# jai1215snu/ShiftedScaleQuantization

Measured on AMD Instinct MI355X. Metric: Gelem/s shifted-scale q/dq + recon iters/s, ResNet-18 W2A4; top-1 vs ref, higher is better.
Workload: dtype f32; 1 GPU; resnet18 W2A4 bias_cal+bias_ch_quant, 1024 calib samples: A4 per-tensor q/dq of act [1024,64,56,56] + W2 per-channel q/dq of all 21 conv/fc weights (8-bit stem/head); parallelism=dp1

## Files before the change

### shiftedscalequantization_amd/csrc/conv_wgrad.hip

```cpp
#include <stdlib.h>

#include <algorithm>
#include <type_traits>

#include "ssq_common.h"

namespace ssq {

typedef float f32x16 __attribute__((ext_vector_type(16)));

constexpr int kUnr = 2;

struct WgradGeo {
  int Nb, C, H, W, Co, OH, OW, R, S, st, pad, G, Cig, Cog;
  int Ncol;
  int WM;
  int Pq;
  int lda;
  int chunks_per_n;
  int nchunks;
  int cps;
  int nsplit;
  int in_rows;
  int ci_span;
// ... 1071 lines not shown
  WgradGeo g;
  size_t lds;
  return wgrad_plan(Nb, C, H, W, Co, R, S, stride, pad, groups, g, &lds) ? 0 : 1;
}

extern "C" size_t ssq_conv_wgrad_workspace_size(int64_t Nb, int64_t C, int64_t H, int64_t W,
                                                int64_t Co, int64_t R, int64_t S, int64_t stride,
                                                int64_t pad, int64_t groups) {
  if (is_depthwise(C, Co, groups) && R * S <= 25 && Nb >= 1 && dw_lds_ok(H, W, pad)) {
    int spl;
    const int ns = dw_splits(Nb, C, &spl);
    const int64_t OH = (H + 2 * pad - R) / stride + 1;
    int64_t nbands = 1;
    if (dw_stage(H, W, pad, spl) == 0 && OH >= 1) {
      const int bh = dw_band_rows(H, W, R, stride, pad, OH);
      nbands = (OH + bh - 1) / bh;
    }
    return (size_t)ns * (size_t)nbands * (size_t)C * (size_t)(R * S) * sizeof(float);
  }
  {
    BandGeo gb;
    int wmx, vpx;
    if (use_band(Nb, C, H, W, Co, R, S, stride, pad, groups, gb, &wmx, &vpx))
      return (size_t)gb.nsplit * 9 * (size_t)Co * (size_t)C * sizeof(float);
  }
  if (use_i2c(R, S, Co, groups)) {
    I2cGeo gi;
    int wm;
    if (wgrad_i2c_plan(Nb, C, H, W, Co, R, S, stride, pad, groups, gi)) return 0;
    wgrad_i2c_tiles(gi, &wm);
    return (size_t)gi.nsplit * (size_t)Co * (size_t)gi.Ncol * sizeof(float);
  }
  if (R == 1 && S == 1 && pad == 0) {
    W1Geo g1;
    if (wgrad_1x1_plan(Nb, C, H, W, Co, stride, groups, g1)) return 0;
    return (size_t)g1.nsplit * (size_t)Co * (size_t)g1.Cig * sizeof(float);
  }
  WgradGeo g;
  size_t lds;
  if (wgrad_plan(Nb, C, H, W, Co, R, S, stride, pad, groups, g, &lds)) return 0;
  return (size_t)g.nsplit * (size_t)Co * (size_t)g.Ncol * sizeof(float);
}

extern "C" int ssq_conv_wgrad(const float* x, const float* dy, int64_t Nb, int64_t C, int64_t H,
                              int64_t W, int64_t Co, int64_t R, int64_t S, int64_t stride,
                              int64_t pad, int64_t groups, float* dw, void* ws, size_t ws_bytes,
                              ssq_stream_t stream) {
  SSQ_REQUIRE(x && dy && dw, SSQ_E_ARG, "ssq_conv_wgrad: null pointer");
  hipStream_t s = (hipStream_t)stream;
  if (is_depthwise(C, Co, groups) && R * S <= 25 && dw_lds_ok(H, W, pad)) {
    SSQ_REQUIRE(Nb >= 1 && H >= 1 && W >= 1 && stride >= 1 && pad >= 0, SSQ_E_ARG,
                "ssq_conv_wgrad: bad geometry");
    const int64_t OH = (H + 2 * pad - R) / stride + 1, OW = (W + 2 * pad - S) / stride + 1;
    SSQ_REQUIRE(OH >= 1 && OW >= 1 && Nb * C * H * W < (1ll << 31) && Nb * C * OH * OW < (1ll << 31),
                SSQ_E_ARG, "ssq_conv_wgrad: sizes");
    int spl;
    const int ns = dw_splits(Nb, C, &spl);
    const size_t need = (size_t)ns * (size_t)C * (size_t)(R * S) * sizeof(float);
    SSQ_REQUIRE(ws && ws_bytes >= need, SSQ_E_WS, "ssq_conv_wgrad: workspace too small");
    const dim3 grid((unsigned)C, (unsigned)ns);
    const int64_t plane = (H + 2 * pad) * (W + 2 * pad);
    const int nb = dw_stage(H, W, pad, spl);
    if (nb > 0) {
      const size_t lds = (size_t)nb * plane * sizeof(float);
      const FastDiv dWp = make_fastdiv((uint32_t)(W + 2 * pad)), dP = make_fastdiv((uint32_t)plane),
                    dOHW = make_fastdiv((uint32_t)(OH * OW)), dOW = make_fastdiv((uint32_t)OW);
      if (R * S <= 9)
        hipLaunchKernelGGL(wgrad_dw_small<9>, grid, dim3(256), lds, s, x, dy, (int)C, (int)H,
                           (int)W, (int)OH, (int)OW, (int)R, (int)S, (int)stride, (int)pad, spl,
                           nb, dWp, dP, dOHW, dOW, (float*)ws);
      else
        hipLaunchKernelGGL(wgrad_dw_small<25>, grid, dim3(256), lds, s, x, dy, (int)C, (int)H,
                           (int)W, (int)OH, (int)OW, (int)R, (int)S, (int)stride, (int)pad, spl,
                           nb, dWp, dP, dOHW, dOW, (float*)ws);
      const int64_t n = C * R * S;
      hipLaunchKernelGGL(wgrad_stage2, dim3((unsigned)std::min<int64_t>((n + 63) / 64, 4096)),
                         dim3(256), 0, s, (const float*)ws, ns, n, dw);
      return check_launch("ssq_conv_wgrad");
    }
    const int bh = dw_band_rows(H, W, R, stride, pad, OH);
    const int nbands = (int)((OH + bh - 1) / bh);
    SSQ_REQUIRE(ws_bytes >= need * (size_t)nbands, SSQ_E_WS, "ssq_conv_wgrad: workspace too small");
    const dim3 gridb((unsigned)C, (unsigned)(ns * nbands));
    const size_t lds = (size_t)(((int64_t)bh - 1) * stride + R) * (W + 2 * pad) * sizeof(float);
    static bool dw_attr = false;
    if (!dw_attr) {
      hipFuncSetAttribute((const void*)wgrad_dw_stage1<9>,
                          hipFuncAttributeMaxDynamicSharedMemorySize, 128 * 1024);
      hipFuncSetAttribute((const void*)wgrad_dw_stage1<25>,
                          hipFuncAttributeMaxDynamicSharedMemorySize, 128 * 1024);
      dw_attr = true;
    }
    if (R * S <= 9)
      hipLaunchKernelGGL(wgrad_dw_stage1<9>, gridb, dim3(256), lds, s, x, dy, (int)C, (int)H, (int)W,
                         (int)OH, (int)OW, (int)R, (int)S, (int)stride, (int)pad, spl, bh, nbands,
                         make_fastdiv((uint32_t)(W + 2 * pad)), (float*)ws);
    else
      hipLaunchKernelGGL(wgrad_dw_stage1<25>, gridb, dim3(256), lds, s, x, dy, (int)C, (int)H, (int)W,
                         (int)OH, (int)OW, (int)R, (int)S, (int)stride, (int)pad, spl, bh, nbands,
                         make_fastdiv((uint32_t)(W + 2 * pad)), (float*)ws);
    const int64_t n = C * R * S;
    hipLaunchKernelGGL(wgrad_stage2, dim3((unsigned)std::min<int64_t>((n + 63) / 64, 4096)),
                       dim3(256), 0, s, (const float*)ws, ns * nbands, n, dw);
    return check_launch("ssq_conv_wgrad");
  }
  {
    BandGeo gb;
    int wmx, vpx;
    if (use_band(Nb, C, H, W, Co, R, S, stride, pad, groups, gb, &wmx, &vpx)) {
      const size_t needb = (size_t)gb.nsplit * 9 * (size_t)Co * (size_t)C * sizeof(float);
      SSQ_REQUIRE(ws && ws_bytes >= needb, SSQ_E_WS, "ssq_conv_wgrad: workspace too small");
      typedef void (*BandK)(const float*, const float*, BandGeo, float*);
#define SSQ_BK(NWV)                                                                          \
  {{{wgrad_band_stage1<2, 1, 4, NWV>, wgrad_band_stage1<2, 1, 2, NWV>,                        \
     wgrad_band_stage1<2, 1, 1, NWV>},                                                        \
    {wgrad_band_stage1<2, 2, 4, NWV>, wgrad_band_stage1<2, 2, 2, NWV>,                        \
     wgrad_band_stage1<2, 2, 1, NWV>}},                                                       \
   {{wgrad_band_stage1<4, 1, 4, NWV>, wgrad_band_stage1<4, 1, 2, NWV>,                        \
     wgrad_band_stage1<4, 1, 1, NWV>},                                                        \
    {wgrad_band_stage1<4, 2, 4, NWV>, wgrad_band_stage1<4, 2, 2, NWV>,                        \
     wgrad_band_stage1<4, 2, 1, NWV>}}}
      static const BandK kernels[2][2][2][3] = {SSQ_BK(4), SSQ_BK(8)};
#undef SSQ_BK
      static bool band_attr = false;
      if (!band_attr) {
        for (auto& a0 : kernels)
          for (auto& a : a0)
            for (auto& b : a)
              for (BandK k : b)
                hipFuncSetAttribute((const void*)k, hipFuncAttributeMaxDynamicSharedMemorySize,
                                    160 * 1024);
        band_attr = true;
      }
      const int w8 = band_waves() == 8;
      const BandK kb = kernels[w8][wmx == 4][stride == 2][vpx == 4 ? 0 : (vpx == 2 ? 1 : 2)];
      const dim3 gridb((unsigned)(gb.nsplit * gb.m_tiles * gb.n_tiles));
      const size_t ldsb = 2 * (size_t)gb.bufsz * sizeof(float);
      hipLaunchKernelGGL(kb, gridb, dim3(w8 ? 512 : 256), ldsb, s, x, dy, gb, (float*)ws);
      const int64_t inner = Co * C, nb = 9 * inner;
      hipLaunchKernelGGL(wgrad_stage2, dim3((unsigned)std::min<int64_t>((nb + 63) / 64, 4096)),
                         dim3(256), 0, s, (const float*)ws, gb.nsplit, nb, dw, inner, 9);
      return check_launch("ssq_conv_wgrad");
    }
  }
  if (use_i2c(R, S, Co, groups)) {
    I2cGeo gi;
    int wm;
    const int rci = wgrad_i2c_plan(Nb, C, H, W, Co, R, S, stride, pad, groups, gi);
    if (rci) return rci;
    wgrad_i2c_tiles(gi, &wm);
    const size_t needi = (size_t)gi.nsplit * (size_t)Co * (size_t)gi.Ncol * sizeof(float);
    SSQ_REQUIRE(ws && ws_bytes >= needi, SSQ_E_WS, "ssq_conv_wgrad: workspace too small");
    const dim3 gridi(gi.n_tiles, gi.m_tiles * gi.G, gi.nsplit);
    (void)wm;
    hipLaunchKernelGGL(wgrad_i2c_stage1<2>, gridi, dim3(256), 0, s, x, dy, gi, (float*)ws);
    const int64_t ni = (int64_t)Co * gi.Ncol;
    hipLaunchKernelGGL(wgrad_stage2, dim3((unsigned)std::min<int64_t>((ni + 63) / 64, 4096)),
                       dim3(256), 0, s, (const float*)ws, gi.nsplit, ni, dw);
    return check_launch("ssq_conv_wgrad");
  }
  if (R == 1 && S == 1 && pad == 0) {
    W1Geo g1;
    const int rc1 = wgrad_1x1_plan(Nb, C, H, W, Co, stride, groups, g1);
    if (rc1) return rc1;
    const size_t need1 = (size_t)g1.nsplit * (size_t)Co * (size_t)g1.Cig * sizeof(float);
    SSQ_REQUIRE(ws && ws_bytes >= need1, SSQ_E_WS, "ssq_conv_wgrad: workspace too small");
    const dim3 grid1(g1.n_tiles, g1.m_tiles * g1.G, g1.nsplit);
    hipLaunchKernelGGL(wgrad_1x1_stage1<2>, grid1, dim3(256), 0, s, x, dy, g1, (float*)ws);
    const int64_t n1 = (int64_t)Co * g1.Cig;
    hipLaunchKernelGGL(wgrad_stage2, dim3((unsigned)std::min<int64_t>((n1 + 63) / 64, 4096)),
                       dim3(256), 0, s, (const float*)ws, g1.nsplit, n1, dw);
    return check_launch("ssq_conv_wgrad");
  }
  WgradGeo g;
  size_t lds;
  int rc = wgrad_plan(Nb, C, H, W, Co, R, S, stride, pad, groups, g, &lds);
  if (rc) return rc;
  const size_t need = (size_t)g.nsplit * (size_t)Co * (size_t)g.Ncol * sizeof(float);
  SSQ_REQUIRE(ws && ws_bytes >= need, SSQ_E_WS, "ssq_conv_wgrad: workspace too small");
  static bool lds_attr = false;
  if (!lds_attr) {
    hipFuncSetAttribute((const void*)wgrad_stage1<1>, hipFuncAttributeMaxDynamicSharedMemorySize,
                        160 * 1024);
    hipFuncSetAttribute((const void*)wgrad_stage1<2>, hipFuncAttributeMaxDynamicSharedMemorySize,
                        160 * 1024);
    hipFuncSetAttribute((const void*)wgrad_stage1<4>, hipFuncAttributeMaxDynamicSharedMemorySize,
                        160 * 1024);
    lds_attr = true;
  }
  const dim3 grid(g.n_tiles, g.m_tiles * g.G, g.nsplit);
  if (g.WM == 1)
    hipLaunchKernelGGL(wgrad_stage1<1>, grid, dim3(256), lds, s, x, dy, g, (float*)ws);
  else if (g.WM == 2)
    hipLaunchKernelGGL(wgrad_stage1<2>, grid, dim3(256), lds, s, x, dy, g, (float*)ws);
  else
    hipLaunchKernelGGL(wgrad_stage1<4>, grid, dim3(256), lds, s, x, dy, g, (float*)ws);
  const int64_t n = (int64_t)Co * g.Ncol;
  hipLaunchKernelGGL(wgrad_stage2, dim3((unsigned)std::min<int64_t>((n + 63) / 64, 4096)),
                     dim3(256), 0, s, (const float*)ws, g.nsplit, n, dw);
  return check_launch("ssq_conv_wgrad");
}

__global__ __launch_bounds__(kBlock) void wgrad_gemm_operands(
    const float* __restrict__ x, const float* __restrict__ dy, uint32_t C, uint32_t H,
    uint32_t W, uint32_t Co, uint32_t R, uint32_t S, uint32_t st, int pad, uint32_t OW,
    uint32_t NP, FastDiv dRS, FastDiv dS, FastDiv dP, FastDiv dOW, uint32_t CRS,
    uint32_t P, uint32_t nb1, uint32_t tiles_k, uint32_t vec4, float* __restrict__ col,
    float* __restrict__ dy2) {
  if (blockIdx.x < nb1) {
    __shared__ float tile[64][65];
    const uint32_t tk = blockIdx.x % tiles_k, tp = blockIdx.x / tiles_k;
    const uint32_t row0 = tp * 64, k0 = tk * 64, RS = R * S;
    const uint32_t pp = threadIdx.x & 63, kb = threadIdx.x >> 6, row = row0 + pp;
    const bool rok = row < NP;
    const uint32_t n = rok ? fdiv(row, dP) : 0u, p = row - n * P;
    const uint32_t oh = fdiv(p, dOW), ow = p - oh * OW;
    const int ih0 = (int)(oh * st) - pad, iw0 = (int)(ow * st) - pad;
    const float* xn = x + (size_t)n * C * H * W;
    float v[16];
#pragma unroll
    for (int j = 0; j < 16; ++j) {
      const uint32_t k = k0 + kb + 4 * j;
      const uint32_t ci = fdiv(k, dRS), rs = k - ci * RS;
      const uint32_t r = fdiv(rs, dS), sc = rs - r * S;
      const int ih = ih0 + (int)r, iw = iw0 + (int)sc;
      v[j] = 0.0f;
      if (rok && k < CRS && ih >= 0 && ih < (int)H && iw >= 0 && iw < (int)W)
        v[j] = xn[((size_t)ci * H + ih) * W + iw];
    }
#pragma unroll
    for (int j = 0; j < 16; ++j) tile[kb + 4 * j][pp] = v[j];
    __syncthreads();
    if (vec4) {
      for (uint32_t i = threadIdx.x; i < 64 * 16; i += kBlock) {
        const uint32_t pp = i >> 4, kq = (i & 15) << 2;
        const uint32_t row = row0 + pp, k = k0 + kq;
        if (row < NP && k < CRS)
          *reinterpret_cast<float4*>(col + (size_t)row * CRS + k) =
              make_float4(tile[kq][pp], tile[kq + 1][pp], tile[kq + 2][pp], tile[kq + 3][pp]);
      }
    } else {
      for (uint32_t i = threadIdx.x; i < 64 * 64; i += kBlock) {
        const uint32_t pp = i >> 6, kk = i & 63;
        const uint32_t row = row0 + pp, k = k0 + kk;
        if (row < NP && k < CRS) col[(size_t)row * CRS + k] = tile[kk][pp];
      }
    }
    return;
  }
  const uint32_t nb2 = gridDim.x - nb1;
  const uint32_t n2 = Co * NP;
  for (uint32_t e = (blockIdx.x - nb1) * kBlock + threadIdx.x; e < n2; e += nb2 * kBlock) {
    const uint32_t co = e / NP, q = e - co * NP;
    const uint32_t n = fdiv(q, dP), p = q - n * P;
    dy2[e] = dy[((size_t)n * Co + co) * P + p];
  }
}

template <int ACT>
__device__ __forceinline__ float epi_in(float v, uint32_t c, const float* __restrict__ bias,
                                        const float* __restrict__ gamma,
                                        const float* __restrict__ phi, bool quant,
                                        const QParams& qp) {
  float t = bias ? __fadd_rn(v, bias[c]) : v;
  if (gamma) t = __fadd_rn(__fmul_rn(t, gamma[c]), phi[c]);
  t = act_fwd<ACT>(t);
  if (quant) {
    float q;
    t = fq1(t, qp, &q);
  }
  return t;
}

template <int ACT>
__global__ __launch_bounds__(kBlock) void gemm_col_epi(
    const float* __restrict__ y, const float* __restrict__ bias, const float* __restrict__ gamma,
    const float* __restrict__ phi, const float* __restrict__ qdelta,
    const float* __restrict__ qzp, float qlo, float qhi, uint32_t C, uint32_t H, uint32_t W,
    uint32_t R, uint32_t S, uint32_t st, int pad, uint32_t OW, uint32_t NP, FastDiv dCRS,
    FastDiv dRS, FastDiv dS, FastDiv dP, FastDiv dOW, uint32_t CRS, uint32_t P,
    float* __restrict__ col) {
  const bool quant = qdelta != nullptr;
  QParams qp{1.0f, 0.0f, qlo, qhi};
  if (quant) {
    qp.d = qdelta[0];
    qp.z = qzp[0];
  }
  const uint32_t n1 = NP * CRS;
  for (uint32_t e = blockIdx.x * kBlock + threadIdx.x; e < n1; e += gridDim.x * kBlock) {
    const uint32_t row = fdiv(e, dCRS), k = e - row * CRS;
    const uint32_t n = fdiv(row, dP), p = row - n * P;
    const uint32_t oh = fdiv(p, dOW), ow = p - oh * OW;
    const uint32_t ci = fdiv(k, dRS), rs = k - ci * R * S;
    const uint32_t r = fdiv(rs, dS), s = rs - r * S;
    const int ih = (int)(oh * st + r) - pad, iw = (int)(ow * st + s) - pad;
    float v = 0.0f;
    if (ih >= 0 && ih < (int)H && iw >= 0 && iw < (int)W)
      v = epi_in<ACT>(y[(((size_t)n * C + ci) * H + ih) * W + iw], ci, bias, gamma, phi, quant,
                      qp);
    col[e] = v;
  }
}

extern "C" int ssq_gemm_col_epilogue(const float* y, const float* bias, const float* gamma,
                                     const float* phi, int relu, const float* delta,
                                     const float* zp, int qmin, int qmax, int64_t Nb, int64_t C,
                                     int64_t H, int64_t W, int64_t R, int64_t S, int64_t stride,
                                     int64_t pad, float* col, ssq_stream_t stream) {
  SSQ_REQUIRE(y && col, SSQ_E_ARG, "ssq_gemm_col_epilogue: null pointer");
  SSQ_REQUIRE(!gamma == !phi, SSQ_E_ARG, "ssq_gemm_col_epilogue: gamma and phi go together");
  SSQ_REQUIRE(!delta || (zp && qmin < qmax), SSQ_E_ARG, "ssq_gemm_col_epilogue: act quantizer");
  SSQ_REQUIRE(relu >= 0 && relu <= 2, SSQ_E_ARG, "ssq_gemm_col_epilogue: activation code %d", relu);
  SSQ_REQUIRE(Nb >= 1 && C >= 1 && H >= 1 && W >= 1 && R >= 1 && S >= 1 && stride >= 1 &&
                  pad >= 0, SSQ_E_ARG, "ssq_gemm_col_epilogue: bad geometry");
  const int64_t OH = (H + 2 * pad - R) / stride + 1, OW = (W + 2 * pad - S) / stride + 1;
  SSQ_REQUIRE(OH >= 1 && OW >= 1, SSQ_E_ARG, "ssq_gemm_col_epilogue: empty output plane");
  const int64_t P = OH * OW, NP = Nb * P, CRS = C * R * S;
  SSQ_REQUIRE(NP * CRS < (1ll << 31) && Nb * C * H * W < (1ll << 31), SSQ_E_ARG,
              "ssq_gemm_col_epilogue: operands exceed 2^31 elements");
  const uint32_t nb = (uint32_t)std::min<int64_t>((NP * CRS + kBlock - 1) / kBlock, 8192);
#define SSQ_GCE(A)                                                                          \
  hipLaunchKernelGGL(gemm_col_epi<A>, dim3(nb), dim3(kBlock), 0, (hipStream_t)stream, y, bias, \
                     gamma, phi, delta, zp, (float)qmin, (float)qmax, (uint32_t)C, (uint32_t)H, \
                     (uint32_t)W, (uint32_t)R, (uint32_t)S, (uint32_t)stride, (int)pad,         \
                     (uint32_t)OW, (uint32_t)NP, make_fastdiv((uint32_t)CRS),                   \
                     make_fastdiv((uint32_t)(R * S)), make_fastdiv((uint32_t)S),                \
                     make_fastdiv((uint32_t)P), make_fastdiv((uint32_t)OW), (uint32_t)CRS,      \
                     (uint32_t)P, col)
  if (relu == 2) SSQ_GCE(2); else if (relu == 1) SSQ_GCE(1); else SSQ_GCE(0);
#undef SSQ_GCE
  return check_launch("ssq_gemm_col_epilogue");
}

extern "C" int ssq_wgrad_gemm_operands(const float* x, const float* dy, int64_t Nb, int64_t C,
                                       int64_t H, int64_t W, int64_t Co, int64_t R, int64_t S,
                                       int64_t stride, int64_t pad, float* col, float* dy2,
                                       ssq_stream_t stream) {
  SSQ_REQUIRE((x && col) || (dy && dy2), SSQ_E_ARG, "ssq_wgrad_gemm_operands: null pointer");
  if (!(x && col)) col = nullptr;
  if (!(dy && dy2)) dy2 = nullptr;
  SSQ_REQUIRE(Nb >= 1 && C >= 1 && H >= 1 && W >= 1 && Co >= 1 && R >= 1 && S >= 1 &&
                  stride >= 1 && pad >= 0, SSQ_E_ARG, "ssq_wgrad_gemm_operands: bad geometry");
  const int64_t OH = (H + 2 * pad - R) / stride + 1, OW = (W + 2 * pad - S) / stride + 1;
  SSQ_REQUIRE(OH >= 1 && OW >= 1, SSQ_E_ARG, "ssq_wgrad_gemm_operands: empty output plane");
  const int64_t P = OH * OW, NP = Nb * P, CRS = C * R * S;
  SSQ_REQUIRE(NP * CRS < (1ll << 31) && Co * NP < (1ll << 31) && Nb * C * H * W < (1ll << 31),
              SSQ_E_ARG, "ssq_wgrad_gemm_operands: operands exceed 2^31 elements");
  const bool vec4 = col && CRS % 4 == 0 && ((uintptr_t)col & 15) == 0;
  const int64_t tiles_k = (CRS + 63) / 64, tiles = ((NP + 63) / 64) * tiles_k;
  SSQ_REQUIRE(tiles < (1ll << 31), SSQ_E_ARG, "ssq_wgrad_gemm_operands: too many tiles");
  const uint32_t nb1 = col ? (uint32_t)tiles : 0u;
  const uint32_t nb2 = dy2 ? (uint32_t)std::min<int64_t>((Co * NP + kBlock - 1) / kBlock, 2048) : 0u;
  hipLaunchKernelGGL(wgrad_gemm_operands, dim3(nb1 + nb2), dim3(kBlock), 0, (hipStream_t)stream,
                     x, dy, (uint32_t)C, (uint32_t)H, (uint32_t)W, (uint32_t)Co, (uint32_t)R,
                     (uint32_t)S, (uint32_t)stride, (int)pad, (uint32_t)OW, (uint32_t)NP,
                     make_fastdiv((uint32_t)(R * S)), make_fastdiv((uint32_t)S),
                     make_fastdiv((uint32_t)P), make_fastdiv((uint32_t)OW), (uint32_t)CRS,
                     (uint32_t)P, nb1, (uint32_t)tiles_k, (uint32_t)vec4, col, dy2);
  return check_launch("ssq_wgrad_gemm_operands");
}
```

Measured before the change: 753.9 Gelem/s.

## Stage input planes in LDS for im2col with fused epilogue and dy repack

Adds a col_staged kernel that loads padded input channel-block bands into shared memory, applies the activation/quant epilogue once per input element, and then emits im2col rows from LDS using vectorized float4 stores. It also folds the dy-to-dy2 repack into the same launch with a vectorized copy path. The goal is to stop re-reading and re-quantizing each input element R*S times from global memory during im2col for wgrad and the GEMM epilogue. In exchange it adds occupancy-sensitive LDS use, env-driven planning heuristics and a fallback for 1x1 or strided cases.

```diff
diff --git a/shiftedscalequantization_amd/csrc/conv_wgrad.hip b/shiftedscalequantization_amd/csrc/conv_wgrad.hip
--- a/shiftedscalequantization_amd/csrc/conv_wgrad.hip
+++ b/shiftedscalequantization_amd/csrc/conv_wgrad.hip
@@ -1397,6 +1397,282 @@
   }
 }
 
+struct ColPlan {
+  uint32_t Nb, C, H, W, R, S, st, OH, OW, P, CRS, RS;
+  int pad;
+  uint32_t CB, NS, BH;
+  uint32_t ncb, nbands;
+  uint32_t Wp, PS;
+  uint32_t vec_in, vec_out;
+  uint32_t nb1;
+  FastDiv dRS, dS, dOW, dBH, dW;
+};
+
+struct Dy2Plan {
+  uint32_t Co, P, NP, chunks, vec;
+  FastDiv dP, dChunks;
+};
+
+struct EpiArgs {
+  const float *bias, *gamma, *phi, *qdelta, *qzp;
+  float qlo, qhi;
+};
+
+constexpr uint32_t kColCB = 32;
+constexpr size_t kColLdsCap = 48 * 1024;
+constexpr size_t kColPlaneCap = 160 * 1024;
+
+template <int EPI>
+__global__ __launch_bounds__(kBlock) void col_staged(const float* __restrict__ x, ColPlan g,
+                                                     EpiArgs ea, float* __restrict__ col,
+                                                     const float* __restrict__ dy, Dy2Plan d,
+                                                     float* __restrict__ dy2) {
+  extern __shared__ __align__(16) float col_lds[];
+  const uint32_t t = threadIdx.x;
+  if (blockIdx.x >= g.nb1) {
+    const uint32_t b2 = blockIdx.x - g.nb1, co = fdiv(b2, d.dChunks);
+    const uint32_t q0 = (b2 - co * d.chunks) * (4 * kBlock);
+    const float* src = dy + (size_t)co * d.P;
+    float* dst = dy2 + (size_t)co * d.NP;
+    if (d.vec) {
+      const uint32_t q = q0 + 4 * t;
+      if (q < d.NP) {
+        const uint32_t n = fdiv(q, d.dP), p = q - n * d.P;
+        *reinterpret_cast<float4*>(dst + q) =
+            *reinterpret_cast<const float4*>(src + (size_t)n * d.Co * d.P + p);
+      }
+    } else {
+#pragma unroll
+      for (int j = 0; j < 4; ++j) {
+        const uint32_t q = q0 + t + kBlock * j;
+        if (q < d.NP) {
+          const uint32_t n = fdiv(q, d.dP), p = q - n * d.P;
+          dst[q] = src[(size_t)n * d.Co * d.P + p];
+        }
+      }
+    }
+    return;
+  }
+  float* pl = col_lds;
+  const uint32_t cbi = blockIdx.x % g.ncb, rest = blockIdx.x / g.ncb;
+  const uint32_t band = rest % g.nbands, sg = rest / g.nbands;
+  const uint32_t cb0 = cbi * g.CB, cbn = min(g.CB, g.C - cb0);
+  const uint32_t n0 = sg * g.NS, nsn = min(g.NS, g.Nb - n0);
+  const uint32_t oh0 = band * g.BH, bhn = min(g.BH, g.OH - oh0);
+  const uint32_t L = cbn * g.RS, nrows = nsn * bhn * g.OW, SS = g.CB * g.PS;
+
+  {
+    const uint32_t n4 = (g.NS * SS + 3) / 4;
+    float4* z = reinterpret_cast<float4*>(pl);
+    for (uint32_t i = t; i < n4; i += kBlock) z[i] = make_float4(0.f, 0.f, 0.f, 0.f);
+  }
+  __syncthreads();
+
+  {
+    const int ih_start = (int)(oh0 * g.st) - g.pad;
+    const int ih_lo = max(ih_start, 0);
+    const int ih_hi = min(ih_start + (int)((bhn - 1) * g.st + g.R), (int)g.H);
+    const uint32_t len = ih_hi > ih_lo ? (uint32_t)(ih_hi - ih_lo) * g.W : 0u;
+    const uint32_t HW = g.H * g.W, first = (uint32_t)ih_lo * g.W;
+    const uint32_t lrow0 = (uint32_t)(ih_lo - ih_start);
+    const bool v4 = g.vec_in && first % 4 == 0 && len % 4 == 0;
+    const uint32_t items = v4 ? len / 4 : len;
+    const uint32_t lg = items <= 16 ? 4u : (items <= 32 ? 5u : 6u);
+    const uint32_t sub = t >> lg, lane = t & ((1u << lg) - 1), nsub = kBlock >> lg;
+    [[maybe_unused]] const bool quant = ea.qdelta != nullptr;
+    [[maybe_unused]] QParams qp{1.0f, 0.0f, ea.qlo, ea.qhi};
+    if constexpr (EPI >= 0) {
+      if (quant) {
+        qp.d = ea.qdelta[0];
+        qp.z = ea.qzp[0];
+      }
+    }
+    constexpr int kU = 8;
+    for (uint32_t ns = 0; ns < nsn; ++ns) {
+      const float* srcn = x + ((size_t)(n0 + ns) * g.C + cb0) * HW + first;
+      float* dstn = pl + ns * SS + lrow0 * g.Wp + (uint32_t)g.pad;
+      for (uint32_t q = lane; q < items; q += 1u << lg) {
+        const uint32_t e0 = v4 ? 4 * q : q;
+        const uint32_t row = fdiv(e0, g.dW), w0 = e0 - row * g.W;
+        for (uint32_t c0 = sub; c0 < cbn; c0 += kU * nsub) {
+          if (v4) {
+            float4 v[kU];
+#pragma unroll
+            for (int u = 0; u < kU; ++u) {
+              const uint32_t c = c0 + u * nsub;
+              if (c < cbn) v[u] = *reinterpret_cast<const float4*>(srcn + (size_t)c * HW + e0);
+            }
+#pragma unroll
+            for (int u = 0; u < kU; ++u) {
+              const uint32_t c = c0 + u * nsub;
+              if (c < cbn) {
+                const float vv[4] = {v[u].x, v[u].y, v[u].z, v[u].w};
+                float* dstp = dstn + c * g.PS;
+                uint32_t rr = row, w = w0;
+#pragma unroll
+                for (int j = 0; j < 4; ++j) {
+                  float e = vv[j];
+                  if constexpr (EPI >= 0)
+                    e = epi_in<(EPI >= 0 ? EPI : 0)>(e, cb0 + c, ea.bias, ea.gamma, ea.phi, quant,
+                                                    qp);
+                  if (w + (uint32_t)g.pad < g.Wp) dstp[rr * g.Wp + w] = e;
+                  if (++w == g.W) {
+                    w = 0;
+                    ++rr;
+                  }
+                }
+              }
+            }
+          } else {
+            float v[kU];
+#pragma unroll
+            for (int u = 0; u < kU; ++u) {
+              const uint32_t c = c0 + u * nsub;
+              if (c < cbn) v[u] = srcn[(size_t)c * HW + e0];
+            }
+#pragma unroll
+            for (int u = 0; u < kU; ++u) {
+              const uint32_t c = c0 + u * nsub;
+              if (c < cbn) {
+                float e = v[u];
+                if constexpr (EPI >= 0)
+                  e = epi_in<(EPI >= 0 ? EPI : 0)>(e, cb0 + c, ea.bias, ea.gamma, ea.phi, quant, qp);
+                if (w0 + (uint32_t)g.pad < g.Wp) dstn[c * g.PS + row * g.Wp + w0] = e;
+              }
+            }
+          }
+        }
+      }
+    }
+  }
+  __syncthreads();
+
+  const uint32_t row0 = n0 * g.P + oh0 * g.OW;
+  float* base = col + (size_t)row0 * g.CRS + cb0 * g.RS;
+  const uint32_t sW = g.st * g.Wp;
+  auto tap = [&](uint32_t k) {
+    const uint32_t c = fdiv(k, g.dRS), rs = k - c * g.RS;
+    const uint32_t r = fdiv(rs, g.dS), s = rs - r * g.S;
+    return c * g.PS + r * g.Wp + s;
+  };
+  uint32_t q, ow, dq, dow;
+  auto seek = [&](uint32_t rl, uint32_t rpt) {
+    q = fdiv(rl, g.dOW), ow = rl - q * g.OW;
+    dq = fdiv(rpt, g.dOW), dow = rpt - dq * g.OW;
+  };
+  auto window = [&]() {
+    const uint32_t ns = fdiv(q, g.dBH), off = ns * SS + (q - ns * g.BH) * sW + ow * g.st;
+    ow += dow, q += dq;
+    if (ow >= g.OW) ow -= g.OW, ++q;
+    return pl + off;
+  };
+  const uint32_t Q = g.vec_out ? L / 4 : 0u;
+  if (Q) {
+    const uint32_t rpt = Q <= kBlock ? kBlock / Q : 1u;
+    const uint32_t rsub = t / Q, jstep = Q <= kBlock ? Q : (uint32_t)kBlock;
+    const size_t dp = (size_t)rpt * g.CRS;
+    for (uint32_t j = t - rsub * Q; j < Q && rsub < rpt; j += jstep) {
+      const uint32_t o0 = tap(4 * j), o1 = tap(4 * j + 1), o2 = tap(4 * j + 2), o3 = tap(4 * j + 3);
+      float* p = base + (size_t)rsub * g.CRS + 4 * j;
+      seek(rsub, rpt);
+      for (uint32_t rl = rsub; rl < nrows; rl += 4 * rpt, p += 4 * dp) {
+        float4 v[4];
+#pragma unroll
+        for (int u = 0; u < 4; ++u) {
+          const float* w = window();
+          if (rl + u * rpt < nrows) v[u] = make_float4(w[o0], w[o1], w[o2], w[o3]);
+        }
+#pragma unroll
+        for (int u = 0; u < 4; ++u)
+          if (rl + u * rpt < nrows) *reinterpret_cast<float4*>(p + u * dp) = v[u];
+      }
+    }
+  }
+  const uint32_t T = L - 4 * Q;
+  if (T) {
+    const uint32_t rpt = T <= kBlock ? kBlock / T : 1u;
+    const uint32_t rsub = t / T, jstep = T <= kBlock ? T : (uint32_t)kBlock;
+    for (uint32_t j = t - rsub * T; j < T && rsub < rpt; j += jstep) {
+      const uint32_t o = tap(4 * Q + j);
+      float* p = base + (size_t)rsub * g.CRS + 4 * Q + j;
+      seek(rsub, rpt);
+      for (uint32_t rl = rsub; rl < nrows; rl += rpt, p += (size_t)rpt * g.CRS) *p = window()[o];
+    }
+  }
+}
+
+static long env_long(const char* name, long dflt) {
+  const char* e = getenv(name);
+  return e && *e ? atol(e) : dflt;
+}
+
+static bool col_plan(int64_t Nb, int64_t C, int64_t H, int64_t W, int64_t R, int64_t S,
+                     int64_t st, int64_t pad, int64_t OH, int64_t OW, const void* src,
+                     const void* col, ColPlan& g, size_t* lds) {
+  const long form = env_long("SSQ_COL_FORM", 1);
+  if (form == 0 || (st != 1 && form != 2)) return false;
+  if (R == 1 && S == 1 && st == 1) return false;
+  const int64_t CB = std::min<int64_t>(kColCB, C), RS = R * S, CRS = C * RS, P = OH * OW;
+  if ((size_t)CB * (H + 2 * pad) * (W + 2 * pad) * sizeof(float) > kColPlaneCap) return false;
+  static int cus = 0;
+  if (!cus) {
+    int dev = 0;
+    if (hipGetDevice(&dev) != hipSuccess ||
+        hipDeviceGetAttribute(&cus, hipDeviceAttributeMultiprocessorCount, dev) != hipSuccess ||
+        cus < 1)
+      cus = 256;
+  }
+  const int64_t target = 2 * (int64_t)cus;
+  const int64_t Wp = ((OW - 1) * st + S + 1) / 2 * 2, ncb = (C + CB - 1) / CB;
+  auto pitch = [&](int64_t bh) { return (((bh - 1) * st + R) * Wp + 2) / 32 * 32 + 29; };
+  auto bytes = [&](int64_t ns, int64_t bh) {
+    return (size_t)((ns * CB * pitch(bh) + 3) / 4 * 4) * sizeof(float);
+  };
+  int64_t NS = 1, nbands = std::min(OH, std::max<int64_t>(1, (target + ncb * Nb - 1) / (ncb * Nb)));
+  int64_t BH = (OH + nbands - 1) / nbands;
+  BH = std::max(BH, std::min(OH, (32 + OW - 1) / OW));
+  while (BH >= 1 && bytes(1, BH) > kColLdsCap) --BH;
+  if (BH < 1) return false;
+  nbands = (OH + BH - 1) / BH;
+  BH = (OH + nbands - 1) / nbands;
+  if (nbands == 1) {
+    const int64_t force = env_long("SSQ_COL_NS", 0);
+    if (force >= 1) {
+      if (bytes(std::min(force, Nb), OH) <= kColLdsCap) NS = std::min(force, Nb);
+    } else {
+      while (2 * NS <= Nb && 2 * NS * P <= 256 && ncb * ((Nb + 2 * NS - 1) / (2 * NS)) >= target &&
+             bytes(2 * NS, OH) <= kColLdsCap)
+        NS *= 2;
+    }
+  }
+  const int64_t nb1 = ncb * nbands * ((Nb + NS - 1) / NS);
+  if (nb1 >= (1ll << 30)) return false;
+  g.Nb = (uint32_t)Nb, g.C = (uint32_t)C, g.H = (uint32_t)H, g.W = (uint32_t)W;
+  g.R = (uint32_t)R, g.S = (uint32_t)S, g.st = (uint32_t)st, g.OH = (uint32_t)OH;
+  g.OW = (uint32_t)OW, g.P = (uint32_t)P, g.CRS = (uint32_t)CRS, g.RS = (uint32_t)RS;
+  g.pad = (int)pad;
+  g.CB = (uint32_t)CB, g.NS = (uint32_t)NS, g.BH = (uint32_t)BH;
+  g.ncb = (uint32_t)ncb, g.nbands = (uint32_t)nbands;
+  g.Wp = (uint32_t)Wp, g.PS = (uint32_t)pitch(BH);
+  g.vec_in = ((uintptr_t)src & 15) == 0 && (H * W) % 4 == 0;
+  g.vec_out = ((uintptr_t)col & 15) == 0 && CRS % 4 == 0 && (CB * RS) % 4 == 0;
+  g.nb1 = (uint32_t)nb1;
+  g.dRS = make_fastdiv((uint32_t)RS), g.dS = make_fastdiv((uint32_t)S);
+  g.dOW = make_fastdiv((uint32_t)OW), g.dBH = make_fastdiv((uint32_t)BH);
+  g.dW = make_fastdiv((uint32_t)W);
+  *lds = bytes(NS, BH);
+  return true;
+}
+
+static Dy2Plan dy2_plan(int64_t Co, int64_t P, int64_t NP, const void* dy, const void* dy2) {
+  Dy2Plan d;
+  d.Co = (uint32_t)Co, d.P = (uint32_t)P, d.NP = (uint32_t)NP;
+  d.chunks = (uint32_t)((NP + 4 * kBlock - 1) / (4 * kBlock));
+  d.vec = P % 4 == 0 && (((uintptr_t)dy | (uintptr_t)dy2) & 15) == 0;
+  d.dP = make_fastdiv((uint32_t)P), d.dChunks = make_fastdiv(d.chunks);
+  return d;
+}
+
 extern "C" int ssq_gemm_col_epilogue(const float* y, const float* bias, const float* gamma,
                                      const float* phi, int relu, const float* delta,
                                      const float* zp, int qmin, int qmax, int64_t Nb, int64_t C,
@@ -1413,6 +1689,18 @@
   const int64_t P = OH * OW, NP = Nb * P, CRS = C * R * S;
   SSQ_REQUIRE(NP * CRS < (1ll << 31) && Nb * C * H * W < (1ll << 31), SSQ_E_ARG,
               "ssq_gemm_col_epilogue: operands exceed 2^31 elements");
+  ColPlan cg;
+  size_t clds;
+  if (col_plan(Nb, C, H, W, R, S, stride, pad, OH, OW, y, col, cg, &clds)) {
+    const EpiArgs ea{bias, gamma, phi, delta, zp, (float)qmin, (float)qmax};
+    const Dy2Plan none{};
+#define SSQ_CSE(A)                                                                          \
+  hipLaunchKernelGGL(col_staged<A>, dim3(cg.nb1), dim3(kBlock), clds, (hipStream_t)stream, y, \
+                     cg, ea, col, (const float*)nullptr, none, (float*)nullptr)
+    if (relu == 2) SSQ_CSE(2); else if (relu == 1) SSQ_CSE(1); else SSQ_CSE(0);
+#undef SSQ_CSE
+    return check_launch("ssq_gemm_col_epilogue");
+  }
   const uint32_t nb = (uint32_t)std::min<int64_t>((NP * CRS + kBlock - 1) / kBlock, 8192);
 #define SSQ_GCE(A)                                                                          \
   hipLaunchKernelGGL(gemm_col_epi<A>, dim3(nb), dim3(kBlock), 0, (hipStream_t)stream, y, bias, \
@@ -1441,6 +1729,23 @@
   const int64_t P = OH * OW, NP = Nb * P, CRS = C * R * S;
   SSQ_REQUIRE(NP * CRS < (1ll << 31) && Co * NP < (1ll << 31) && Nb * C * H * W < (1ll << 31),
               SSQ_E_ARG, "ssq_wgrad_gemm_operands: operands exceed 2^31 elements");
+  ColPlan cg{};
+  size_t clds = 0;
+  Dy2Plan d{};
+  if (dy2) d = dy2_plan(Co, P, NP, dy, dy2);
+  const long form = env_long("SSQ_COL_FORM", 1);
+  if (form != 0 && (col ? col_plan(Nb, C, H, W, R, S, stride, pad, OH, OW, x, col, cg, &clds)
+                        : (d.vec || form == 2))) {
+    uint32_t nb2s = 0;
+    if (dy2) {
+      SSQ_REQUIRE(Co * (int64_t)d.chunks < (1ll << 30), SSQ_E_ARG,
+                  "ssq_wgrad_gemm_operands: too many tiles");
+      nb2s = (uint32_t)Co * d.chunks;
+    }
+    hipLaunchKernelGGL(col_staged<-1>, dim3(cg.nb1 + nb2s), dim3(kBlock), clds,
+                       (hipStream_t)stream, x, cg, EpiArgs{}, col, dy, d, dy2);
+    return check_launch("ssq_wgrad_gemm_operands");
+  }
   const bool vec4 = col && CRS % 4 == 0 && ((uintptr_t)col & 15) == 0;
   const int64_t tiles_k = (CRS + 63) / 64, tiles = ((NP + 63) / 64) * tiles_k;
   SSQ_REQUIRE(tiles < (1ll << 31), SSQ_E_ARG, "ssq_wgrad_gemm_operands: too many tiles");
```

After: 753.3 Gelem/s. Within noise of the previous version (-0.1%).
